# ucsdmanorlab/bootstrapper

Measured on AMD Instinct MI355X. Metric: Mvoxels/s predict+segment, 1024^3 vol in 128^3 blocks, higher is better.
Workload: dtype bf16x3

## Files before the change

### bootstrapper_amd/csrc/unet_api.hip

```cpp
#include <algorithm>
#include <cmath>
#include <cstdlib>
#include <cstring>
#include <map>
#include <memory>
#include <mutex>
#include <vector>
#include <chrono>
#include <thread>

#include "unet_internal.h"
#include "unet_ops.h"

#include "dev_guard.h"

namespace bsmi {

static thread_local std::string g_err;
void set_error(const char* fmt, ...) {
  char buf[1024];
  va_list ap;
  va_start(ap, fmt);
  vsnprintf(buf, sizeof buf, fmt, ap);
  va_end(ap);
// ... 170 lines not shown
        } else {
          const uint16_t hi = host_f32_to_bf16(v);
          const uint16_t lo = host_f32_to_bf16(v - host_bf16_to_f32(hi));
          uint16_t* w16 = (uint16_t*)packed.data();
          if (fused) {
            w16[idx] = hi;
            w16[idx + nelem] = lo;
          } else {
            const size_t blk = (size_t)pc.Npad * BKE;
            w16[idx] = hi;
            w16[idx + blk] = hi;
            w16[idx + 2 * blk] = lo;
          }
        }
      }
    }
  });
  BSMI_HIP(hipMalloc(&pc.w, packed.size()));
  BSMI_HIP(hipMemcpy(pc.w, packed.data(), packed.size(), hipMemcpyHostToDevice));
  BSMI_HIP(hipMalloc((void**)&pc.bias, bias.size() * sizeof(float)));
  BSMI_HIP(hipMemcpy(pc.bias, bias.data(), bias.size() * sizeof(float), hipMemcpyHostToDevice));
  pc.ready = true;
  return BSMI_OK;
}

static int wino_mode() {
  static const int m = [] { const char* e = getenv("BSMI_WINO"); return e ? atoi(e) : 1; }();
  return m;
}
static int wino4_mode();
static bool wino_eligible(const PassSite& p, int ci) {
  if (wino_mode() == 0 || p.k[ci][0] != 3 || p.k[ci][1] != 3 || p.k[ci][2] != 3) return false;
  if (ci == 0 && p.nslots > kWinoMaxSrc) return false;
  if (!x3_fused_for(choose_tile(p.cout))) return false;
  if (wino_mode() >= 2) return true;
  int cin = p.cout;
  if (ci == 0) {
    cin = 0;
    for (int s = 0; s < p.nslots; ++s) cin += p.cin[s];
  }
  if (cin >= 256 && p.cout >= 256) return true;
  return wino4_mode() == 1 && (int64_t)cin * p.cout >= 16384 && cin >= 32 && p.cout >= 32;
}

static int wino4_mode() {
  static const int m = [] { const char* e = getenv("BSMI_WINO4"); return e ? atoi(e) : 1; }();
  return m;
}
static int wino_tile_edge(const PassSite& p, int ci) {
  (void)p; (void)ci;
  return wino4_mode() == 0 ? 2 : 4;
}

static int pack_wino(bsmi_unet* h, PassSite& p, int ci) {
  PackedWino& pw = p.wino[ci];
  if (pw.w) { (void)hipFree(pw.w); pw.w = nullptr; }
  if (pw.res_w) { (void)hipFree(pw.res_w); pw.res_w = nullptr; }
  for (int part = 0; part < 2; ++part)
    if (pw.res_part_w[part]) { (void)hipFree(pw.res_part_w[part]); pw.res_part_w[part] = nullptr; }
  pw.ready = false;
  if (!wino_eligible(p, ci)) return BSMI_OK;
  const HostWeight& wm = h->weights[p.prefix + ".conv_pass." + std::to_string(2 * ci) + ".weight"];
  const HostWeight& wr = h->weights[p.prefix + ".residual.0.weight"];
  const int cin_m = (int)wm.shape[1];
  pw.cin_of_v.clear();
  if (ci == 0) {
    int base = 0;
    for (int s = 0; s < p.nslots; ++s) {
      for (int c = 0; c < round_up(p.cin[s], kChanPad); ++c) pw.cin_of_v.push_back(c < p.cin[s] ? base + c : -1);
      base += p.cin[s];
    }
  } else {
    for (int c = 0; c < round_up(p.cout, kChanPad); ++c) pw.cin_of_v.push_back(c < p.cout ? c : -1);
  }
  pw.Cv = (int)pw.cin_of_v.size();
  pw.m = wino_tile_edge(p, ci);
  pw.tile = choose_tile(p.cout);
  pw.Npad = round_up(p.cout, tile_bn(pw.tile));
  wino_units(pw.Cv, pw.units);
  {
    size_t image_elems = 0, batch_elems = 0;
    static const bool on_host = [] { const char* e = getenv("BSMI_WINO_PACK_HOST"); return e && e[0] == '1'; }();
    if (on_host) {
      std::vector<uint16_t> packed;
      wino_pack_weights(wm.data.data(), p.cout, cin_m, pw.cin_of_v, pw.Npad, pw.units, packed, image_elems, batch_elems, pw.m);
      BSMI_HIP(hipMalloc(&pw.w, packed.size() * 2));
      BSMI_HIP(hipMemcpy(pw.w, packed.data(), packed.size() * 2, hipMemcpyHostToDevice));
    } else {
      const int rc = wino_pack_weights_dev(wm.data.data(), p.cout, cin_m, pw.cin_of_v, pw.Npad, pw.units, pw.m, &pw.w, image_elems, batch_elems);
      if (rc) return rc;
    }
    pw.lo_image_bytes = image_elems * 2;
    pw.batch_bytes = batch_elems * 2;
  }
  pw.res_entries.clear();
  if (ci == p.nconv - 1) {
    std::vector<PackEntry> all;
    build_entries(p, ci, BSMI_PREC_BF16X3, all);
    for (size_t u = 0; u + 1 < all.size(); u += kUnitsPerStep) {
      bool res = false;
      for (int j = 0; j < kUnitsPerStep; ++j) res |= !all[u + j].dummy && all[u + j].wsrc == 1;
      if (res)
        for (int j = 0; j < kUnitsPerStep; ++j) pw.res_entries.push_back(all[u + j]);
    }
    if ((pw.res_entries.size() / kUnitsPerStep) % 2)
      for (int j = 0; j < kUnitsPerStep; ++j) pw.res_entries.push_back(PackEntry{0, 0, 0, 0, 0, 0, 0, 0, 0, true, 0});
    const int64_t cin_r = wr.shape[1];
    auto pack_res = [&](const std::vector<PackEntry>& ents, void** w_out, size_t* lo_out) -> int {
      const size_t nsteps = ents.size() / kUnitsPerStep;
      const size_t nelem = (nsteps * (size_t)pw.Npad + kWeightRowSlack) * 32;
      std::vector<uint16_t> packed(2 * nelem, 0);
      for (size_t u = 0; u < ents.size(); ++u) {
        const PackEntry& e = ents[u];
        if (e.dummy) continue;
// ... 403 lines not shown
            }
      }
    }
    const int n_full = (int)chunks.size();
    for (const Src& sr : center) {
      const TDesc& t = slots[sr.slot];
      const int org[3] = {so[sr.slot][0] + crop[0] / 2, so[sr.slot][1] + crop[1] / 2, so[sr.slot][2] + crop[2] / 2};
      for (int c0 = 0; c0 < t.Cpad; c0 += 32) {
        chunks.push_back(chunk_of(t, org, c0));
        const size_t w0 = wimg.size();
        wimg.resize(w0 + (size_t)NB * 64 * 4, 0u);
        for (int b = 0; b < NB; ++b)
          for (int l = 0; l < 64; ++l) {
            const int m = b * 16 + (l & 15), q = l >> 4;
            if (m >= p.cout) continue;
            for (int j = 0; j < 8; ++j) {
              const int c = c0 + q * 8 + j;
              if (c >= sr.creal) break;
              put(w0 + ((size_t)b * 64 + l) * 4, j, wr.data[(size_t)m * cin_r + (sr.cin_base + c)]);
            }
          }
      }
    }
    std::vector<float> bias((size_t)16 * NB, 0.f);
    for (int m = 0; m < p.cout; ++m) bias[m] = bm.data[m] + (last ? br.data[m] : 0.f);
    BoxChunk* dchunks = nullptr;
    uint32_t* dw = nullptr;
    float* dbias = nullptr;
    BSMI_HIP(hipMalloc((void**)&dchunks, chunks.size() * sizeof(BoxChunk)));
    plan->allocs.push_back(dchunks);
    BSMI_HIP(hipMalloc((void**)&dw, wimg.size() * 4));
    plan->allocs.push_back(dw);
    BSMI_HIP(hipMalloc((void**)&dbias, bias.size() * 4));
    plan->allocs.push_back(dbias);
    BSMI_HIP(hipMemcpy(dchunks, chunks.data(), chunks.size() * sizeof(BoxChunk), hipMemcpyHostToDevice));
    BSMI_HIP(hipMemcpy(dw, wimg.data(), wimg.size() * 4, hipMemcpyHostToDevice));
    BSMI_HIP(hipMemcpy(dbias, bias.data(), bias.size() * 4, hipMemcpyHostToDevice));
    st.box.chunks = dchunks;
    st.box.n_full = n_full;
    st.box.n_center = (int)chunks.size() - n_full;
    st.box.w = dw;
    st.box.bias = dbias;
    st.box.out = (uint16_t*)o.ptr;
    st.box.Do = o.D; st.box.Ho = o.H; st.box.Wo = o.W; st.box.Co = o.Cpad;
    st.use_box = true;
    (void)nsl;
    return BSMI_OK;
  }

  int plan_wino(PassSite& p, int ci, const PackedConv& pc, const TDesc* slots, const int (*so)[3], int nsl, const TDesc& o, PlanStep& st) {
    st.use_wino = false;
    const PackedWino& pw = p.wino[ci];
    const bool wants_fused = fuse_up && (ci == 0 || ci == p.nconv - 1);
    const int wm = pw.m, nbatch = wino_batches(wm);
    if (prec != BSMI_PREC_BF16X3 || !pw.ready || (wm == 2 && ((o.H & 1) || (o.W & 1))) || st.use_box || st.use_rh) {
      if (wants_fused) BSMI_FAIL(BSMI_ERR_STATE, "%s conv %d: the upsampling was fused into this stage, which cannot take the Winograd form", p.prefix.c_str(), ci);
      return BSMI_OK;
    }
    const int nsrc = ci == 0 ? p.nslots : 1;
    const int Dv = o.D + 2, Ty = (o.H + wm - 1) / wm, Tx = (o.W + wm - 1) / wm, Cv = pw.Cv;
    const size_t vbatch = (size_t)Dv * Ty * Tx * Cv * 4;
    if (vbatch >= ((size_t)1 << 31)) {
      if (wants_fused) BSMI_FAIL(BSMI_ERR_STATE, "%s conv %d: fused upsampling, but the transformed input is too large", p.prefix.c_str(), ci);
      return BSMI_OK;
    }
    const size_t Mrows = (size_t)o.D * Ty * Tx;
    void *V = nullptr, *Mbuf = nullptr, *addend = nullptr;
    BSMI_HIP(hipMalloc(&V, nbatch * vbatch + 4096));
    plan->allocs.push_back(V);
    BSMI_HIP(hipMalloc(&Mbuf, nbatch * Mrows * o.Cpad * sizeof(float)));
    plan->allocs.push_back(Mbuf);
    plan->bytes += nbatch * (vbatch + Mrows * o.Cpad * sizeof(float));
    WinoInArgs& wi = st.wino_in;
    memset(&wi, 0, sizeof wi);
    int cv0 = 0;
    for (int q = 0; q < nsrc; ++q) {
      const TDesc& t = slots[q];
      wi.src[q] = t.ptr;
      wi.H[q] = t.H; wi.W[q] = t.W; wi.Cpad[q] = t.Cpad;
      wi.oz[q] = so[q][0]; wi.oy[q] = so[q][1]; wi.ox[q] = so[q][2];
      wi.cv0[q] = cv0;
      cv0 += t.Cpad;
      if (fuse_up && ci == 0 && q == 1) {
        if (fuse_up->low.Cpad != t.Cpad) BSMI_FAIL(BSMI_ERR_STATE, "%s: fused upsampling with a different channel padding", p.prefix.c_str());
        wi.src[q] = fuse_up->low.ptr;
        wi.H[q] = fuse_up->low.H; wi.W[q] = fuse_up->low.W;
        wi.oz[q] += fuse_up->o[0]; wi.oy[q] += fuse_up->o[1]; wi.ox[q] += fuse_up->o[2];
        wi.upf[q] = fuse_up->f[1];
      }
    }
    if (cv0 != Cv) BSMI_FAIL(BSMI_ERR_STATE, "%s conv %d: winograd channel layout %d != %d", p.prefix.c_str(), ci, cv0, Cv);
    wi.nsrc = nsrc;
    wi.V = V;
    wi.Dv = Dv; wi.Ty = Ty; wi.Tx = Tx; wi.Cv = Cv;
    wi.m = wm;
    ConvArgs& g = st.wino_gemm;
    memset(&g, 0, sizeof g);
    for (int sl = 0; sl < kMaxConvTensors; ++sl) {
      g.t[sl].base = (uint64_t)(uintptr_t)V;
      g.t[sl].sz = (int32_t)((int64_t)Ty * Tx * Cv * 4);
      g.t[sl].sy = (int32_t)((int64_t)Tx * Cv * 4);
      g.t[sl].sx = (int32_t)((int64_t)Cv * 4);
    }
    {
      std::vector<KStep> ks(pw.units.size() / kUnitsPerStep);
      for (size_t s = 0; s < ks.size(); ++s) {
// ... 257 lines not shown
        }
        st.out = o;
        rc = plan_rh(p, ci, pc, slots, so, nsl, o, st);
        if (rc) return rc;
        rc = plan_box(p, ci, slots, so, nsl, o, st);
        if (rc) return rc;
        rc = plan_wino(p, ci, pc, slots, so, nsl, o, st);
        if (rc) return rc;
        if (!st.use_wino && !st.use_box) {
          rc = plan_h16(p, ci, pc, slots, so, o, st);
          if (rc) return rc;
        }
        if (getenv("BSMI_PLAN_DEBUG"))
          fprintf(stderr, "[bsmi plan] %s conv %d: out (%d,%d,%d)x%d tile BN=%d K-steps %d %s\n", p.prefix.c_str(), ci, o.D, o.H, o.W,
                  p.cout, tile_bn(st.tile), st.use_wino ? st.wino_gemm.nsteps : a.nsteps,
                  st.use_wino ? (st.wino_in.m == 4 ? "winograd F(4x4,3x3)" : "winograd F(2x2,3x3)") : st.use_h16 ? "halo-resident" : st.use_box ? "box-halo" : st.use_rh ? "raster-halo" : "gather");
        plan->steps.push_back(st);
      }
      cur = o;
      sp[0] = o.D; sp[1] = o.H; sp[2] = o.W;
    }
    out = cur;
    (void)crop;
    return BSMI_OK;
  }

  int rec(int level, const TDesc& f_in, TDesc& f_out) {
    const int i = h->nl - level - 1;
    TDesc f_left;
    const int org0[1][3] = {{0, 0, 0}};
    const int sp[3] = {f_in.D, f_in.H, f_in.W};
    int rc = pass(h->l_conv[i], &f_in, org0, sp, f_left);
    if (rc) return rc;
    if (level == 0) {
      f_out = f_left;
      return BSMI_OK;
    }
    const int* f = h->cfg.downsample_factors[i];
    const int dims[3] = {f_left.D, f_left.H, f_left.W};
    for (int d = 2; d >= 0; --d)
      if (dims[d] % f[d] != 0)
        BSMI_FAIL(BSMI_ERR_INVALID,
                  "Can not downsample shape (%d, %d, %d) with factor (%d, %d, %d), mismatch in spatial dimension %d",
                  dims[0], dims[1], dims[2], f[0], f[1], f[2], d);
    TDesc g_in;
    g_in.C = f_left.C; g_in.D = f_left.D / f[0]; g_in.H = f_left.H / f[1]; g_in.W = f_left.W / f[2];
    rc = alloc(g_in);
    if (rc) return rc;
    if (!dry) {
      PlanStep st;
      st.type = PlanStep::POOL;
      st.in = f_left; st.out = g_in;
      for (int d = 0; d < 3; ++d) st.f[d] = f[d];
      plan->steps.push_back(st);
    }
    TDesc g_out;
    rc = rec(level - 1, g_in, g_out);
    if (rc) return rc;

    PassSite& rp = h->r_conv[i];
    const int up[3] = {g_out.D * f[0], g_out.H * f[1], g_out.W * f[2]};
    int conv_crop[3] = {0, 0, 0};
    for (int c = 0; c < rp.nconv; ++c)
      for (int d = 0; d < 3; ++d) conv_crop[d] += rp.k[c][d] - 1;
    int target[3];
    for (int d = 0; d < 3; ++d) {
      const int cf = h->crop_factor[i][d];
      const int n = (int)std::floor((double)(up[d] - conv_crop[d]) / cf);
      target[d] = n * cf + conv_crop[d];
      if (target[d] != up[d] && target[d] <= conv_crop[d])
        BSMI_FAIL(BSMI_ERR_INVALID,
                  "Feature map with shape (%d, %d, %d) is too small to ensure translation equivariance",
                  up[0], up[1], up[2]);
    }
    TDesc g_c;
    g_c.C = g_out.C; g_c.D = target[0]; g_c.H = target[1]; g_c.W = target[2];
    rc = alloc(g_c);
    if (rc) return rc;
    int so[2][3];
    for (int d = 0; d < 3; ++d) {
      so[0][d] = (dims[d] - target[d]) / 2;
      so[1][d] = 0;
      if (dims[d] < target[d])
        BSMI_FAIL(BSMI_ERR_INVALID, "skip connection (%d,%d,%d) smaller than upsampled map (%d,%d,%d)",
                  dims[0], dims[1], dims[2], target[0], target[1], target[2]);
    }
    UpFuse uf;
    bool fuse = false;
    if (!dry && prec == BSMI_PREC_BF16X3 && f[0] == 1 && f[1] == 2 && f[2] == 2 && rp.nslots == 2 && rp.wino[0].ready &&
        rp.wino[rp.nconv - 1].ready && !rp.wino[rp.nconv - 1].res_part[1].empty() && g_out.ptr) {
      static const bool on = [] { const char* e = getenv("BSMI_FUSE_UP"); return !(e && e[0] == '0'); }();
      fuse = on;
      int sp[3] = {target[0], target[1], target[2]};
      for (int c = 0; c < rp.nconv && fuse; ++c) {
        for (int d = 0; d < 3; ++d) sp[d] -= rp.k[c][d] - 1;
        const int wm = rp.wino[c].m;
        if ((c == 0 || c == rp.nconv - 1) && ((wm == 2 && ((sp[1] & 1) || (sp[2] & 1))) || sp[0] <= 0 || sp[1] <= 0 || sp[2] <= 0)) fuse = false;
        if ((c == 0 || c == rp.nconv - 1) && (size_t)(sp[0] + 2) * ((sp[1] + wm - 1) / wm) * ((sp[2] + wm - 1) / wm) * rp.wino[c].Cv * 4 >= ((size_t)1 << 31)) fuse = false;
      }
    }
    size_t up_index = 0;
    if (!dry) {
      PlanStep st;
      st.type = PlanStep::UP;
      st.in = g_out; st.out = g_c;
      for (int d = 0; d < 3; ++d) { st.f[d] = f[d]; st.o[d] = (up[d] - target[d]) / 2; }
// ... 19 lines not shown
    x.C = h->cfg.in_channels; x.D = (int)in_shape[0]; x.H = (int)in_shape[1]; x.W = (int)in_shape[2];
    int rc = alloc(x);
    if (rc) return rc;
    if (!dry) {
      PlanStep st;
      st.type = PlanStep::INPUT;
      st.out = x;
      plan->steps.push_back(st);
    }
    TDesc z;
    rc = rec(h->nl - 1, x, z);
    if (rc) return rc;
    plan->out_shape[0] = z.D; plan->out_shape[1] = z.H; plan->out_shape[2] = z.W;
    for (size_t hd = 0; hd < h->heads.size(); ++hd) {
      plan->flops += 2.0 * 2.0 * (double)z.D * z.H * z.W * h->heads[hd].cin * h->heads[hd].cout;
      if (!dry) {
        PlanStep st;
        st.type = PlanStep::HEAD;
        st.in = z;
        st.head = (int)hd;
        st.flops = 2.0 * 2.0 * (double)z.D * z.H * z.W * h->heads[hd].cin * h->heads[hd].cout;
        plan->steps.push_back(st);
      }
    }
    return BSMI_OK;
  }
};

static void free_plan(Plan* p) {
  for (void* a : p->allocs) (void)hipFree(a);
  p->allocs.clear();
  for (auto* sets : {&p->inflight, &p->spare})
    for (auto& set : *sets)
      for (hipEvent_t e : set) (void)hipEventDestroy(e);
  p->inflight.clear();
  p->spare.clear();
  p->events.clear();
}

static int harvest(bsmi_unet* h, Plan* plan) {
  if (!plan || plan->inflight.empty()) return BSMI_OK;
  const size_t n = plan->steps.size();
  for (auto& set : plan->inflight) {
    plan->last_ms.assign(n, 0.f);
    BSMI_HIP(hipEventSynchronize(set[2 * n - 1]));
    for (size_t i = 0; i < n; ++i) {
      float t = 0.f;
      BSMI_HIP(hipEventElapsedTime(&t, set[2 * i], set[2 * i + 1]));
      plan->last_ms[i] = t;
      const int ty = (plan->fused_first && i < 2) ? (int)PlanStep::CONV : (int)plan->steps[i].type;
      h->prof_ms[ty] += t;
      h->prof_flops[ty] += plan->steps[i].flops;
      if (ty == 1) h->prof_exec += plan->steps[i].exec_flops > 0 ? plan->steps[i].exec_flops : plan->steps[i].flops * (plan->prec == BSMI_PREC_BF16X3 ? 3.0 : 1.0);
      h->prof_launches[ty] += (plan->fused_first && i < 2) ? 0 : 1;
    }
    plan->spare.push_back(std::move(set));
  }
  plan->inflight.clear();
  plan->pending = false;
  return BSMI_OK;
}

namespace {
std::mutex g_chain_mu;
struct ChainState { hipEvent_t done = nullptr; hipStream_t last = nullptr; bool any = false; };
ChainState g_chain[16];
}
struct ForwardChain {
  std::unique_lock<std::mutex> lock{g_chain_mu};
};
static bool forward_chain_on() {
  static const bool on = [] { const char* e = getenv("BSMI_FORWARD_CHAIN"); return e && e[0] == '1'; }();
  return on;
}
static int forward_chain_enter(int device, hipStream_t s) {
  if (device < 0 || device >= 16 || !forward_chain_on()) return BSMI_OK;
  ChainState& c = g_chain[device];
  if (c.any && c.last != s) BSMI_HIP(hipStreamWaitEvent(s, c.done, 0));
  return BSMI_OK;
}
static int forward_chain_leave(int device, hipStream_t s) {
  if (device < 0 || device >= 16 || !forward_chain_on()) return BSMI_OK;
  ChainState& c = g_chain[device];
  if (!c.done) BSMI_HIP(hipEventCreateWithFlags(&c.done, hipEventDisableTiming));
  BSMI_HIP(hipEventRecord(c.done, s));
  c.last = s;
  c.any = true;
  return BSMI_OK;
}

static bool first_pass_eligible(const bsmi_unet* h) {
  if (h->cfg.in_channels != 1 || h->l_conv.empty()) return false;
  const PassSite& p = h->l_conv[0];
  if (p.nconv != 2 || p.cout > 16) return false;
  for (int c = 0; c < 2; ++c)
    for (int d = 0; d < 3; ++d)
      if (p.k[c][d] != 3) return false;
  const char* e = getenv("BSMI_FUSED_FIRST");
  return !(e && e[0] == '0');
}

int get_plan(bsmi_unet* h, int precision, const int64_t in_shape[3], Plan** out) {
  const std::vector<int64_t> key = {precision, in_shape[0], in_shape[1], in_shape[2]};
  auto it = h->plans.find(key);
  if (it == h->plans.end()) {
    std::unique_ptr<Plan> plan(new Plan);
    plan->prec = precision;
    Planner pl{h, precision, plan.get(), false};
    const int rc = pl.run(in_shape);
    if (rc) {
      free_plan(plan.get());
      return rc;
    }
    const std::vector<PlanStep>& ps = plan->steps;
    const bool fp_ready = precision == BSMI_PREC_BF16 ? h->first_pass.ready : precision == BSMI_PREC_BF16X3 && h->first_pass_x3.ready;
    plan->fused_first = fp_ready && first_pass_eligible(h) && ps.size() > 3 &&
                        ps[0].type == PlanStep::INPUT && ps[1].type == PlanStep::CONV && ps[2].type == PlanStep::CONV &&
                        ps[1].site == &h->l_conv[0] && ps[2].site == &h->l_conv[0] && ps[2].out.Cpad == 16;
    BSMI_HIP(hipDeviceSynchronize());
    it = h->plans.emplace(key, std::move(plan)).first;
  }
  *out = it->second.get();
  return BSMI_OK;
}

static int check_shape_arg(const int64_t s[3]) {
  for (int d = 0; d < 3; ++d)
    if (s[d] <= 0 || s[d] > 4096) BSMI_FAIL(BSMI_ERR_INVALID, "bad input shape (%lld,%lld,%lld)", (long long)s[0], (long long)s[1], (long long)s[2]);
  return BSMI_OK;
}

}

extern "C" {

const char* bsmi_last_error(void) { return g_err.c_str(); }
int bsmi_version(void) { return 1; }

int bsmi_unet_create(const bsmi_unet_config* cfg, int device, bsmi_unet** out) {
  if (!cfg || !out) BSMI_FAIL(BSMI_ERR_INVALID, "null argument");
  if (cfg->num_levels < 1 || cfg->num_levels > BSMI_MAX_LEVELS) BSMI_FAIL(BSMI_ERR_INVALID, "num_levels %d out of range", cfg->num_levels);
  if (cfg->num_heads < 1 || cfg->num_heads > BSMI_MAX_HEADS) BSMI_FAIL(BSMI_ERR_INVALID, "num_heads %d out of range", cfg->num_heads);
  if (cfg->in_channels < 1 || cfg->num_fmaps < 1 || cfg->fmap_inc_factor < 1 || cfg->num_fmaps_out < 0) BSMI_FAIL(BSMI_ERR_INVALID, "bad channel configuration");
  std::unique_ptr<bsmi_unet> h(new bsmi_unet);
  h->cfg = *cfg;
  h->device = device;
  h->nl = cfg->num_levels;
  auto fm = [&](int level) {
    int64_t c = cfg->num_fmaps;
    for (int i = 0; i < level; ++i) c *= cfg->fmap_inc_factor;
    return (int)c;
  };
  auto fill_k = [&](PassSite& p, int n, const int32_t (*k)[3]) -> int {
    if (n < 1 || n > BSMI_MAX_CONVS) BSMI_FAIL(BSMI_ERR_INVALID, "%s: %d convolutions per pass unsupported", p.prefix.c_str(), n);
    p.nconv = n;
    for (int i = 0; i < n; ++i)
      for (int d = 0; d < 3; ++d) {
        if (k[i][d] < 1 || k[i][d] > 7) BSMI_FAIL(BSMI_ERR_INVALID, "%s: kernel size %d unsupported", p.prefix.c_str(), k[i][d]);
        p.k[i][d] = k[i][d];
      }
    return BSMI_OK;
  };
  for (int l = 0; l < h->nl; ++l) {
    PassSite p;
    p.prefix = "unet.l_conv." + std::to_string(l);
    p.nslots = 1;
    p.cin[0] = l == 0 ? cfg->in_channels : fm(l - 1);
    p.cout = fm(l);
    int rc = fill_k(p, cfg->n_convs_down[l], cfg->kernel_size_down[l]);
    if (rc) return rc;
    h->l_conv.push_back(p);
// ... 264 lines not shown
    const char* e = getenv("BSMI_STREAMK");
    if ((e && e[0] == '0') || h->sk_request == 0) {
      h->sk_grid = -1;
    } else {
      hipDeviceProp_t prop;
      BSMI_HIP(hipGetDeviceProperties(&prop, h->device));
      h->sk_grid = h->sk_request >= 0 ? h->sk_request : prop.multiProcessorCount / 8 * 8;
      if (const char* g = getenv("BSMI_SK_GRID")) h->sk_grid = std::max(8, atoi(g) / 8 * 8);
      BSMI_HIP(hipMalloc((void**)&h->sk_ws, stream_k_ws_bytes(h->sk_grid)));
      BSMI_HIP(hipMemsetAsync((char*)h->sk_ws + stream_k_ws_bytes(h->sk_grid) - 64, 0, 64, s));
    }
  }
  if (h->train && precision == BSMI_PREC_F32 && !h->train_forward && (rc = train_refresh_f32_images(h, s))) return rc;
  size_t step_idx = 0;
  for (const PlanStep& st : plan.steps) {
    if (prof) BSMI_HIP(hipEventRecord(plan.events[2 * step_idx], s));
    if (plan.fused_first && step_idx < 3) {
      if (step_idx == 2) {
        FirstPassArgs fa;
        fa.raw = raw_dev; fa.raw_dtype = raw_dtype;
        fa.D = plan.steps[0].out.D; fa.H = plan.steps[0].out.H; fa.W = plan.steps[0].out.W;
        fa.out = (uint16_t*)st.out.ptr;
        const FirstPassWeights& fw = precision == BSMI_PREC_BF16X3 ? h->first_pass_x3 : h->first_pass;
        fa.w1a = fw.w1a; fa.w2a = fw.w2a; fa.vec = fw.vec;
        fa.split = fw.split;
        rc = launch_first_pass(fa, h->sk_grid > 0 ? h->sk_grid : 256, s);
        if (rc) return rc;
      }
      if (prof) BSMI_HIP(hipEventRecord(plan.events[2 * step_idx + 1], s));
      ++step_idx;
      continue;
    }
    switch (st.type) {
      case PlanStep::INPUT:
        rc = launch_input_prep(precision, raw_dev, raw_dtype, st.out.ptr, st.out.C, st.out.Cpad,
                               (size_t)st.out.D * st.out.H * st.out.W, s);
        break;
      case PlanStep::CONV:
        if (st.use_wino && !(st.tx3 && h->train_forward)) {
          if ((rc = launch_wino_in(st.wino_in, s))) break;
          if ((rc = launch_conv_igemm(st.wino_gemm, precision, st.tile, s, h->sk_ws, h->sk_grid))) break;
          if (st.wino_has_res && (rc = launch_conv_igemm(st.wino_res, precision, st.tile, s, h->sk_ws, h->sk_grid))) break;
          if (st.wino_has_res_low && (rc = launch_conv_igemm(st.wino_res_low, precision, st.tile, s, h->sk_ws, h->sk_grid))) break;
          rc = launch_wino_out(st.wino_out, s);
          break;
        }
        rc = (st.tx3 && h->train_forward) ? train_forward_conv_x3(h, st, s)
             : st.use_h16 ? launch_conv_h16(st.h16, st.h16_rows, s)
             : st.use_box ? launch_conv_box(st.box, s)
             : st.use_rh ? launch_conv_rh(st.rh, precision, st.tile, s, h->sk_ws, h->sk_grid)
                         : launch_conv_igemm(st.conv, precision, st.tile, s, h->sk_ws, h->sk_grid);
        break;
      case PlanStep::POOL:
        rc = launch_maxpool(precision, st.in.ptr, st.out.ptr, st.in.D, st.in.H, st.in.W, st.in.Cpad,
                            st.f[0], st.f[1], st.f[2], s);
        break;
      case PlanStep::UP:
        if (st.skip) break;
        rc = launch_upsample_crop(precision, st.in.ptr, st.out.ptr, st.in.D, st.in.H, st.in.W, st.in.Cpad,
                                  st.out.D, st.out.H, st.out.W, st.f[0], st.f[1], st.f[2], st.o[0], st.o[1], st.o[2], s);
        break;
      case PlanStep::HEAD: {
        const HeadSite& hd = h->heads[st.head];
        float* of = out_f32_dev ? out_f32_dev[st.head] : nullptr;
        uint8_t* ou = out_u8_dev ? out_u8_dev[st.head] : nullptr;
        if (of || ou)
          rc = launch_head(precision, st.in.ptr, st.in.Cpad, hd.cin, hd.cout, hd.hw, hd.hb, of, ou,
                           (size_t)st.in.D * st.in.H * st.in.W, s);
        break;
      }
    }
    if (rc) return rc;
    if (prof) BSMI_HIP(hipEventRecord(plan.events[2 * step_idx + 1], s));
    ++step_idx;
  }
  if (prof) plan.inflight.push_back(std::move(plan.events));
  return forward_chain_leave(h->device, s);
}

int bsmi_unet_debug_activation(bsmi_unet* h, int step, int what, int64_t shape_out[4], float* host_out, uint64_t capacity) {
  if (!h || !shape_out) BSMI_FAIL(BSMI_ERR_INVALID, "null argument");
  Plan* plan = h->last_plan;
  if (!plan) BSMI_FAIL(BSMI_ERR_STATE, "no forward has run");
  if (step < 0 || step >= (int)plan->steps.size()) BSMI_FAIL(BSMI_ERR_INVALID, "step %d out of range (%zu steps)", step, plan->steps.size());
  const PlanStep& st = plan->steps[step];
  if (st.type == PlanStep::HEAD) BSMI_FAIL(BSMI_ERR_INVALID, "head steps write into the caller's buffers");
  if (plan->fused_first && step < 2)
    BSMI_FAIL(BSMI_ERR_STATE, "step %d is not materialised: the first ConvPass ran as one launch (first_pass), which writes step 2 only", step);
  if (st.type == PlanStep::UP && st.skip)
    BSMI_FAIL(BSMI_ERR_STATE, "step %d is not materialised: the upsampling is fused into the Winograd stages that read it", step);
  const TDesc& t = st.out;
  shape_out[0] = t.D; shape_out[1] = t.H; shape_out[2] = t.W; shape_out[3] = t.C;
  if (!host_out) return BSMI_OK;
  const size_t nvox = (size_t)t.D * t.H * t.W;
  if (capacity < nvox * t.C) BSMI_FAIL(BSMI_ERR_INVALID, "buffer of %llu floats too small", (unsigned long long)capacity);
  BSMI_HIP(hipSetDevice(h->device));
  BSMI_HIP(hipDeviceSynchronize());
  const int es = esize(plan->prec);
  const bool split = t.lo_off != 0;
  const size_t bytes = nvox * t.Cpad * es * (split ? 2 : 1);
  std::vector<uint8_t> raw(bytes);
  BSMI_HIP(hipMemcpy(raw.data(), t.ptr, raw.size(), hipMemcpyDeviceToHost));
  for (size_t v = 0; v < nvox; ++v)
    for (int c = 0; c < t.C; ++c) {
      float x;
      if (plan->prec == BSMI_PREC_F32) {
// ... 130 lines not shown
```

### bootstrapper_amd/csrc/unet_internal.h

```cpp
#pragma once
#include <map>
#include <memory>
#include <string>
#include <vector>

#include "conv_igemm.h"
#include "conv_rh.h"
#include "conv_h16.h"
#include "conv_box.h"
#include "first_pass.h"
#include "wino.h"

namespace bsmi {

struct HostWeight {
  std::vector<int64_t> shape;
  std::vector<float> data;
  bool loaded = false;
};

struct PackEntry {
  int slot;
  int dz, dy, dx;
  int c0;
  int wsrc;
  int tap;
  int cin_base;
  int creal;
  bool dummy;
  int phase;
};

struct PackPhase {
  int slot, c0, kind, first_unit, nunits;
};

struct PackedConv {
  bool ready = false;
  std::vector<PackEntry> entries;
  std::vector<PackPhase> phases;
  void* w = nullptr;
  int ks = 1;
  size_t lo_image_bytes = 0;
  float* bias = nullptr;
  int Npad = 0;
  TileCfg tile = TILE_256x32;
};

struct PackedWino {
  bool ready = false;
  int m = 2;
  std::vector<WinoUnit> units;
  std::vector<int> cin_of_v;
  int Cv = 0;
  void* w = nullptr;
  size_t lo_image_bytes = 0, batch_bytes = 0;
  int Npad = 0;
  TileCfg tile = TILE_256x32;
  std::vector<PackEntry> res_entries;
  void* res_w = nullptr;
  size_t res_lo_image_bytes = 0;
  std::vector<PackEntry> res_part[2];
  void* res_part_w[2] = {nullptr, nullptr};
  size_t res_part_lo[2] = {0, 0};
};

struct H16PhaseHost {
  int slot, c0, dz, kind;
  int first_step, nsteps;
};
struct PackedH16 {
  bool ready = false;
  std::vector<PackEntry> entries;
  std::vector<H16PhaseHost> phases;
  void* w = nullptr;
  size_t lo_image_bytes = 0;
  int Npad = 0;
};

struct PassSite {
  std::string prefix;
  int nslots = 1;
  int cin[2] = {0, 0};
  int cout = 0;
  int nconv = 0;
  int k[BSMI_MAX_CONVS][3];
  PackedConv packed[BSMI_NUM_PREC][BSMI_MAX_CONVS];
  PackedWino wino[BSMI_MAX_CONVS];
  PackedH16 h16[BSMI_MAX_CONVS];
};

struct HeadSite {
  std::string prefix;
  int cin = 0, cout = 0;
  float* hw = nullptr;
  float* hb = nullptr;
};

struct TDesc {
  void* ptr = nullptr;
  int C = 0, Cpad = 0, D = 0, H = 0, W = 0;
  size_t lo_off = 0;
};

struct PlanStep {
  enum Type { INPUT, CONV, POOL, UP, HEAD } type;
  ConvArgs conv;
  RhArgs rh;
  bool use_rh = false;
  H16Args h16;
  bool use_h16 = false;
  int h16_rows = 0;
  BoxArgs box;
  bool use_box = false;
  bool use_wino = false;
  WinoInArgs wino_in;
  ConvArgs wino_gemm, wino_res, wino_res_low;
  bool wino_has_res = false, wino_has_res_low = false;
  WinoOutArgs wino_out;
  TileCfg tile;
  TDesc in, out;
  int f[3], o[3];
  bool skip = false;
  int head = 0;
  double flops = 0;
  double exec_flops = 0;
  struct PassSite* site = nullptr;
  int ci = 0;
  TDesc slots[kMaxConvTensors];
  int so[kMaxConvTensors][3] = {{0, 0, 0}, {0, 0, 0}, {0, 0, 0}};
  int nsl = 0;
  struct TrainFwdX3* tx3 = nullptr;
};

struct Plan {
  std::vector<float> last_ms;
  bool pending = false;
  std::vector<void*> allocs;
  std::vector<PlanStep> steps;
  int64_t out_shape[3] = {0, 0, 0};
  double flops = 0;
  size_t bytes = 0;
  std::vector<hipEvent_t> events;
  std::vector<std::vector<hipEvent_t>> inflight, spare;
  bool profiled = false;
  bool fused_first = false;
  int prec = 0;
};

struct TrainState;

int esize(int prec);
int ksplit(int prec);
int bke(int prec);
int sube(int prec);
void build_entries(const PassSite& p, int ci, int prec, std::vector<PackEntry>& out, std::vector<PackPhase>* phases_out = nullptr);

}

using namespace bsmi;

struct bsmi_unet {
  bsmi_unet_config cfg;
  int device = 0;
  int nl = 0;
  std::vector<PassSite> l_conv, r_conv;
  std::vector<HeadSite> heads;
  int crop_factor[BSMI_MAX_LEVELS][3];
  std::map<std::string, HostWeight> weights;
  bool finalized[BSMI_NUM_PREC] = {false, false, false};
  int profile_period = 0;
  uint64_t profile_count = 0;
  Plan* last_plan = nullptr;
  double prof_ms[5] = {0, 0, 0, 0, 0}, prof_flops[5] = {0, 0, 0, 0, 0};
  double prof_exec = 0;
  int64_t prof_launches[5] = {0, 0, 0, 0, 0};
// ... 19 lines not shown
```

### bootstrapper_amd/csrc/wino.h

```cpp
#pragma once
#include <vector>

#include "conv_igemm.h"

namespace bsmi {

constexpr int kWinoBatch = 16;
constexpr int kWinoMaxBatch = 36;
inline int wino_batches(int m) { return (m + 2) * (m + 2); }
constexpr int kWinoMaxSrc = 2;

struct WinoInArgs {
  const void* src[kWinoMaxSrc];
  int H[kWinoMaxSrc], W[kWinoMaxSrc], Cpad[kWinoMaxSrc];
  int oz[kWinoMaxSrc], oy[kWinoMaxSrc], ox[kWinoMaxSrc];
  int cv0[kWinoMaxSrc];
  int upf[kWinoMaxSrc];
  int nsrc;
  void* V;
  int Dv, Ty, Tx, Cv;
  int m;
};

struct WinoOutArgs {
  const float* M;
  const float* addend;
  const float* low;
  int lD, lH, lW, lf, loz, loy, lox;
  const float* bias;
  void* out;
  int Do, Ty, Tx, Co;
  int relu;
  int m, Ho, Wo;
};

int launch_wino_in(const WinoInArgs& a, hipStream_t s);
int launch_wino_out(const WinoOutArgs& a, hipStream_t s);

struct WinoUnit {
  int kz, vc0;
  bool dummy;
};
void wino_units(int Cv, std::vector<WinoUnit>& out);

void wino_pack_weights(const float* w, int cout, int cin, const std::vector<int>& cin_of_v, int Npad, const std::vector<WinoUnit>& units,
                       std::vector<uint16_t>& packed, size_t& image_elems, size_t& batch_elems, int m = 2);

int wino_pack_weights_dev(const float* w, int cout, int cin, const std::vector<int>& cin_of_v, int Npad, const std::vector<WinoUnit>& units, int m,
                          void** image_dev, size_t& image_elems, size_t& batch_elems);

}
```

### bootstrapper_amd/csrc/wino.hip

```cpp
#include "wino.h"

#include <cstdlib>
#include <cstring>

#include "dev_guard.h"

namespace bsmi {

typedef uint32_t u32x4_t __attribute__((ext_vector_type(4)));
typedef float f32x4_t __attribute__((ext_vector_type(4)));

namespace {

__device__ __forceinline__ uint16_t to_bf16(float f) {
  __bf16 h = (__bf16)f;
  return __builtin_bit_cast(uint16_t, h);
}
__device__ __forceinline__ void unpack8(u32x4_t v, float* f) {
  const uint32_t w[4] = {v.x, v.y, v.z, v.w};
#pragma unroll
  for (int i = 0; i < 4; ++i) {
    f[2 * i] = __uint_as_float(w[i] << 16);
    f[2 * i + 1] = __uint_as_float(w[i] & 0xffff0000u);
  }
// ... 454 lines not shown
  const size_t e_out = (((size_t)z * a.Ty + ty) * a.Tx) * a.Cv + a.cv0[src] + 8 * cv;
  float ct[5][6][4];
  auto load_ct = [&](int c, int xlow) __attribute__((always_inline)) {
    const int x = xlow < 0 ? 0 : (xlow > W - 1 ? W - 1 : xlow);
    float L[5][4];
#pragma unroll
    for (int k = 0; k < 5; ++k) load_split4(sp, e_low + ((size_t)wy[k] * W + x) * C, hf, L[k]);
#pragma unroll
    for (int xi = 0; xi < 6; ++xi)
#pragma unroll
      for (int ch = 0; ch < 4; ++ch) {
        float acc = 0.f;
#pragma unroll
        for (int k = 0; k < 5; ++k)
          if (tu4(PY, xi, k) != 0.f) acc += tu4(PY, xi, k) * L[k][ch];
        ct[c][xi][ch] = acc;
      }
  };
  load_ct(0, bx + 2 * tx0);
  load_ct(1, bx + 2 * tx0 + 1);
  load_ct(2, bx + 2 * tx0 + 2);
  uint16_t* vt = (uint16_t*)a.V + 2 * (e_out + (size_t)tx0 * a.Cv) + 8 * hf;
  for (int tx = tx0; tx < tx1; ++tx) {
    load_ct(3, bx + 2 * tx + 3);
    load_ct(4, bx + 2 * tx + 4);
    uint16_t* vp = vt;
#pragma unroll
    for (int xi = 0; xi < 6; ++xi) {
#pragma unroll
      for (int nu = 0; nu < 6; ++nu) {
        float v[4];
#pragma unroll
        for (int ch = 0; ch < 4; ++ch) {
          float acc = 0.f;
#pragma unroll
          for (int c = 0; c < 5; ++c)
            if (tu4(PX, nu, c) != 0.f) acc += tu4(PX, nu, c) * ct[c][xi][ch];
          v[ch] = acc;
        }
        store_split4_pair(vp, hf, v);
        vp += 2 * plane;
      }
    }
    vt += 2 * a.Cv;
#pragma unroll
    for (int c = 0; c < 3; ++c)
#pragma unroll
      for (int xi = 0; xi < 6; ++xi)
#pragma unroll
        for (int ch = 0; ch < 4; ++ch) ct[c][xi][ch] = ct[c + 2][xi][ch];
  }
}

template <bool LOW>
__global__ __launch_bounds__(256) void wino4_out_kernel(const WinoOutArgs a, size_t total) {
  const size_t i = (size_t)blockIdx.x * blockDim.x + threadIdx.x;
  if (i >= total) return;
  const int ncg = a.Co >> 2;
  const int cg = (int)(i % ncg), cv = cg >> 1, hf = cg & 1;
  size_t t = i / ncg;
  const int tx = (int)(t % a.Tx);
  t /= a.Tx;
  const int ty = (int)(t % a.Ty);
  const int z = (int)(t / a.Ty);
  const size_t Mrows = (size_t)a.Do * a.Ty * a.Tx;
  const size_t m = ((size_t)z * a.Ty + ty) * a.Tx + tx;
  float tp[6][4][4];
#pragma unroll
  for (int nu = 0; nu < 6; ++nu) {
    float mm[6][4];
#pragma unroll
    for (int xi = 0; xi < 6; ++xi) {
      const f32x4_t v = __builtin_nontemporal_load((const f32x4_t*)(a.M + ((size_t)(6 * xi + nu) * Mrows + m) * a.Co + 4 * cg));
#pragma unroll
      for (int k = 0; k < 4; ++k) mm[xi][k] = v[k];
    }
    at4_apply(mm, tp[nu]);
  }
  float bv[4];
#pragma unroll
  for (int k = 0; k < 4; ++k) bv[k] = a.bias[4 * cg + k];
  uint16_t* out = (uint16_t*)a.out;
#pragma unroll
  for (int p = 0; p < 4; ++p) {
    float in[6][4], y[4][4];
#pragma unroll
    for (int nu = 0; nu < 6; ++nu)
#pragma unroll
      for (int k = 0; k < 4; ++k) in[nu][k] = tp[nu][p][k];
    at4_apply(in, y);
    const int oy = 4 * ty + p;
    if (oy >= a.Ho) continue;
#pragma unroll
    for (int q = 0; q < 4; ++q) {
      const int ox = 4 * tx + q;
      if (ox >= a.Wo) continue;
      const size_t e8 = (((size_t)z * a.Ho + oy) * a.Wo + ox) * a.Co + 8 * cv;
      const size_t e = e8 + 4 * hf;
      float v[4];
#pragma unroll
      for (int k = 0; k < 4; ++k) v[k] = y[q][k] + bv[k];
      if (a.addend) {
        const f32x4_t r0 = __builtin_nontemporal_load((const f32x4_t*)(a.addend + e));
#pragma unroll
        for (int k = 0; k < 4; ++k) v[k] += r0[k];
      }
      if constexpr (LOW) {
        int y0, y1, x0, x1;
        float wy0, wy1, wx0, wx1;
        lin_src(oy + a.loy, a.lf, a.lH, y0, y1, wy0, wy1);
        lin_src(ox + a.lox, a.lf, a.lW, x0, x1, wx0, wx1);
        const float* base = a.low + ((size_t)(z + a.loz) * a.lH * a.lW) * a.Co + 4 * cg;
        const f32x4_t r00 = *(const f32x4_t*)(base + ((size_t)y0 * a.lW + x0) * a.Co), r01 = *(const f32x4_t*)(base + ((size_t)y0 * a.lW + x1) * a.Co);
        const f32x4_t r10 = *(const f32x4_t*)(base + ((size_t)y1 * a.lW + x0) * a.Co), r11 = *(const f32x4_t*)(base + ((size_t)y1 * a.lW + x1) * a.Co);
#pragma unroll
        for (int k = 0; k < 4; ++k) {
          const float pa = wx0 * r00[k] + wx1 * r01[k];
          const float pb = wx0 * r10[k] + wx1 * r11[k];
          v[k] += wy0 * pa + wy1 * pb;
        }
      }
      if (a.relu) {
#pragma unroll
        for (int k = 0; k < 4; ++k) v[k] = v[k] > 0.f ? v[k] : 0.f;
      }
      store_split4(out, e8, hf, v);
    }
  }
}

}

static int wino_in_seg_mode() {
  static const int m = [] { const char* e = getenv("BSMI_WINO_IN_SEG"); return e ? atoi(e) : -1; }();
  return m;
}
static void wino_in_segments(int Tx, int& S, int& nseg) {
  const int mode = wino_in_seg_mode();
  S = mode < 0 ? 1 : mode == 0 ? Tx : mode < Tx ? mode : Tx;
  nseg = (Tx + S - 1) / S;
}

int launch_wino_in(const WinoInArgs& a, hipStream_t s) {
  const int m = a.m == 4 ? 4 : 2;
  if (a.m != 0 && a.m != 2 && a.m != 4) BSMI_FAIL(BSMI_ERR_INVALID, "winograd input transform: tile edge %d (2 or 4)", a.m);
  if (a.nsrc < 1 || a.nsrc > kWinoMaxSrc || a.Dv <= 0 || a.Ty <= 0 || a.Tx <= 0 || a.Cv % 8) BSMI_FAIL(BSMI_ERR_INVALID, "winograd input transform: bad geometry");
  for (int q = 0; q < a.nsrc; ++q) {
    if (a.Cpad[q] % 8 || a.cv0[q] % 8 || a.cv0[q] + a.Cpad[q] > a.Cv) BSMI_FAIL(BSMI_ERR_INVALID, "winograd input transform: bad channel layout of source %d", q);
    const int upf = a.upf[q] > 0 ? a.upf[q] : 1;
    if (m == 2 && (a.oy[q] + 2 * a.Ty + 2 > a.H[q] * upf || a.ox[q] + 2 * a.Tx + 2 > a.W[q] * upf)) BSMI_FAIL(BSMI_ERR_INVALID, "winograd input transform: tiles leave source %d", q);
    if (m == 4 && (a.oy[q] < 0 || a.ox[q] < 0 || a.oy[q] + 4 * a.Ty + 2 > a.H[q] * upf + 3 || a.ox[q] + 4 * a.Tx + 2 > a.W[q] * upf + 3))
      BSMI_FAIL(BSMI_ERR_INVALID, "winograd input transform: F(4x4) tiles leave source %d by more than a tile's overhang", q);
    int S = a.Tx, nseg = 1;
    if (m == 4) wino_in_segments(a.Tx, S, nseg);
    const size_t total = (size_t)a.Dv * a.Ty * (a.Cpad[q] / (m == 4 ? 4 : 8)) * nseg;
    const dim3 grid((unsigned)((total + 255) / 256));
    if (a.upf[q] > 0) {
      if (a.upf[q] != 2 || a.oy[q] < 0 || a.ox[q] < 0) BSMI_FAIL(BSMI_ERR_INVALID, "winograd input transform: only a factor-2 upsampling can be fused");
      const int par = 2 * (a.oy[q] & 1) + (a.ox[q] & 1);
      if (m == 4) {
        if (par == 0) hipLaunchKernelGGL((wino4_in_up_kernel<0, 0>), grid, dim3(256), 0, s, a, q, total, S, nseg);
        else if (par == 1) hipLaunchKernelGGL((wino4_in_up_kernel<0, 1>), grid, dim3(256), 0, s, a, q, total, S, nseg);
        else if (par == 2) hipLaunchKernelGGL((wino4_in_up_kernel<1, 0>), grid, dim3(256), 0, s, a, q, total, S, nseg);
        else hipLaunchKernelGGL((wino4_in_up_kernel<1, 1>), grid, dim3(256), 0, s, a, q, total, S, nseg);
      } else if (par == 0) hipLaunchKernelGGL((wino_in_up_kernel<0, 0>), grid, dim3(256), 0, s, a, q, total);
      else if (par == 1) hipLaunchKernelGGL((wino_in_up_kernel<0, 1>), grid, dim3(256), 0, s, a, q, total);
      else if (par == 2) hipLaunchKernelGGL((wino_in_up_kernel<1, 0>), grid, dim3(256), 0, s, a, q, total);
      else hipLaunchKernelGGL((wino_in_up_kernel<1, 1>), grid, dim3(256), 0, s, a, q, total);
    } else if (m == 4) {
      hipLaunchKernelGGL(wino4_in_kernel, grid, dim3(256), 0, s, a, q, total, S, nseg);
    } else {
      hipLaunchKernelGGL(wino_in_kernel, grid, dim3(256), 0, s, a, q, total);
    }
  }
  BSMI_HIP(hipGetLastError());
  return BSMI_OK;
}

int launch_wino_out(const WinoOutArgs& a, hipStream_t s) {
  const int m = a.m == 4 ? 4 : 2;
  if (a.m != 0 && a.m != 2 && a.m != 4) BSMI_FAIL(BSMI_ERR_INVALID, "winograd output transform: tile edge %d (2 or 4)", a.m);
  if (a.Do <= 0 || a.Ty <= 0 || a.Tx <= 0 || a.Co % 8) BSMI_FAIL(BSMI_ERR_INVALID, "winograd output transform: bad geometry");
  const int Ho = m == 4 ? a.Ho : 2 * a.Ty, Wo = m == 4 ? a.Wo : 2 * a.Tx;
  if (m == 4 && (Ho < 1 || Wo < 1 || Ho > 4 * a.Ty || Wo > 4 * a.Tx || Ho + 3 < 4 * a.Ty || Wo + 3 < 4 * a.Tx)) BSMI_FAIL(BSMI_ERR_INVALID, "winograd output transform: output extent and F(4x4) tile counts disagree");
  if (a.low && (a.lf < 1 || a.loz < 0 || a.loz + a.Do > a.lD || a.loy < 0 || a.loy + Ho > a.lH * a.lf || a.lox < 0 || a.lox + Wo > a.lW * a.lf))
    BSMI_FAIL(BSMI_ERR_INVALID, "winograd output transform: the low-resolution residual does not cover the output");
  const size_t total = (size_t)a.Do * a.Ty * a.Tx * (a.Co / (m == 4 ? 4 : 8));
  const dim3 grid((unsigned)((total + 255) / 256));
  if (m == 4) {
    if (a.low) hipLaunchKernelGGL(wino4_out_kernel<true>, grid, dim3(256), 0, s, a, total);
    else hipLaunchKernelGGL(wino4_out_kernel<false>, grid, dim3(256), 0, s, a, total);
  } else if (a.low) hipLaunchKernelGGL(wino_out_kernel<true>, grid, dim3(256), 0, s, a, total);
  else hipLaunchKernelGGL(wino_out_kernel<false>, grid, dim3(256), 0, s, a, total);
  BSMI_HIP(hipGetLastError());
  return BSMI_OK;
}

void wino_units(int Cv, std::vector<WinoUnit>& out) {
  out.clear();
  for (int c32 = 0; c32 < Cv; c32 += 32)
    for (int kz = 0; kz < 3; ++kz)
      for (int j = 0; j < kUnitsPerStep; ++j) {
        const int c = c32 + 16 * j;
        if (c < Cv) out.push_back(WinoUnit{kz, c, false});
        else out.push_back(WinoUnit{0, 0, true});
      }
  if ((out.size() / kUnitsPerStep) % 2)
    for (int j = 0; j < kUnitsPerStep; ++j) out.push_back(WinoUnit{0, 0, true});
}

static inline uint16_t host_bf16(float f) {
  uint32_t u;
  memcpy(&u, &f, 4);
  if ((u & 0x7fffffffu) > 0x7f800000u) return (uint16_t)((u >> 16) | 0x40);
  u += 0x7fffu + ((u >> 16) & 1u);
  return (uint16_t)(u >> 16);
}
static inline float host_bf16_f32(uint16_t b) {
  const uint32_t u = (uint32_t)b << 16;
  float f;
  memcpy(&f, &u, 4);
  return f;
}

void wino_pack_weights(const float* w, int cout, int cin, const std::vector<int>& cin_of_v, int Npad, const std::vector<WinoUnit>& units,
                       std::vector<uint16_t>& packed, size_t& image_elems, size_t& batch_elems, int m) {
  const size_t nsteps = units.size() / kUnitsPerStep;
  const int T = m + 2, nbatch = T * T;
  batch_elems = nsteps * (size_t)Npad * 32;
  image_elems = nbatch * batch_elems + (size_t)kWeightRowSlack * 32;
  packed.assign(2 * image_elems, 0);
  static const double G2[4][3] = {{1, 0, 0}, {.5, .5, .5}, {.5, -.5, .5}, {0, 0, 1}};
  const double a = 0.70710678118654752440, b = 1.41421356237309504880;
  const double G4[6][3] = {{1, 0, 0}, {2. / 3, 2. / 3 * a, 1. / 3}, {2. / 3, -2. / 3 * a, 1. / 3}, {1. / 12, b / 12, 1. / 6}, {1. / 12, -b / 12, 1. / 6}, {0, 0, 1}};
  double G[6][3];
  for (int i = 0; i < T; ++i)
    for (int k = 0; k < 3; ++k) G[i][k] = m == 4 ? G4[i][k] : G2[i][k];
  host_parallel_for((size_t)cout, [&](size_t n_) {
    const int n = (int)n_;
    for (size_t u = 0; u < units.size(); ++u) {
      const WinoUnit& un = units[u];
      if (un.dummy) continue;
      const size_t s = u / kUnitsPerStep, j = u % kUnitsPerStep;
// ... 116 lines not shown
```

Before: 105.8.

## Fuse 1x2x2 max-pool into Winograd F(4x4) output transform and enable narrow last conv Winograd

After: 108.9, median of 6. 3.0% higher.

```diff
diff --git a/bootstrapper_amd/csrc/unet_api.hip b/bootstrapper_amd/csrc/unet_api.hip
--- a/bootstrapper_amd/csrc/unet_api.hip
+++ b/bootstrapper_amd/csrc/unet_api.hip
@@ -246,6 +246,19 @@
   return wino4_mode() == 0 ? 2 : 4;
 }
 
+static bool fuse_up_narrow() {
+  static const bool on = [] { const char* e = getenv("BSMI_FUSE_UP_NARROW"); return !(e && e[0] == '0'); }();
+  return on;
+}
+static bool wino_narrow_last(const bsmi_unet* h, const PassSite& p, int ci) {
+  if (!fuse_up_narrow() || wino_mode() == 0 || p.nslots != 2 || p.nconv < 2 || ci != p.nconv - 1) return false;
+  if (&p < h->r_conv.data() || &p >= h->r_conv.data() + h->r_conv.size()) return false;
+  const int* f = h->cfg.downsample_factors[&p - h->r_conv.data()];
+  if (f[0] != 1 || f[1] != 2 || f[2] != 2) return false;
+  if (p.k[ci][0] != 3 || p.k[ci][1] != 3 || p.k[ci][2] != 3 || p.cout < 32 || !x3_fused_for(choose_tile(p.cout))) return false;
+  return wino_eligible(p, 0) && !wino_eligible(p, ci);
+}
+
 static int pack_wino(bsmi_unet* h, PassSite& p, int ci) {
   PackedWino& pw = p.wino[ci];
   if (pw.w) { (void)hipFree(pw.w); pw.w = nullptr; }
@@ -253,7 +266,8 @@
   for (int part = 0; part < 2; ++part)
     if (pw.res_part_w[part]) { (void)hipFree(pw.res_part_w[part]); pw.res_part_w[part] = nullptr; }
   pw.ready = false;
-  if (!wino_eligible(p, ci)) return BSMI_OK;
+  pw.fused_only = wino_narrow_last(h, p, ci);
+  if (!wino_eligible(p, ci) && !pw.fused_only) return BSMI_OK;
   const HostWeight& wm = h->weights[p.prefix + ".conv_pass." + std::to_string(2 * ci) + ".weight"];
   const HostWeight& wr = h->weights[p.prefix + ".residual.0.weight"];
   const int cin_m = (int)wm.shape[1];
@@ -763,6 +777,7 @@
     st.use_wino = false;
     const PackedWino& pw = p.wino[ci];
     const bool wants_fused = fuse_up && (ci == 0 || ci == p.nconv - 1);
+    if (pw.fused_only && !fuse_up) return BSMI_OK;
     const int wm = pw.m, nbatch = wino_batches(wm);
     if (prec != BSMI_PREC_BF16X3 || !pw.ready || (wm == 2 && ((o.H & 1) || (o.W & 1))) || st.use_box || st.use_rh) {
       if (wants_fused) BSMI_FAIL(BSMI_ERR_STATE, "%s conv %d: the upsampling was fused into this stage, which cannot take the Winograd form", p.prefix.c_str(), ci);
@@ -1126,6 +1141,13 @@
       st.type = PlanStep::POOL;
       st.in = f_left; st.out = g_in;
       for (int d = 0; d < 3; ++d) st.f[d] = f[d];
+      static const bool pool_fuse = [] { const char* e = getenv("BSMI_POOL_FUSE"); return !(e && e[0] == '0'); }();
+      PlanStep& prod = plan->steps.back();
+      if (pool_fuse && prec == BSMI_PREC_BF16X3 && f[0] == 1 && f[1] == 2 && f[2] == 2 && prod.type == PlanStep::CONV && prod.use_wino &&
+          prod.wino_out.m == 4 && !prod.wino_out.low && prod.wino_out.out == f_left.ptr && !(f_left.H & 1) && !(f_left.W & 1)) {
+        prod.wino_out.pool = g_in.ptr;
+        st.pool_fused = true;
+      }
       plan->steps.push_back(st);
     }
     TDesc g_out;
@@ -1251,7 +1273,7 @@
       h->prof_ms[ty] += t;
       h->prof_flops[ty] += plan->steps[i].flops;
       if (ty == 1) h->prof_exec += plan->steps[i].exec_flops > 0 ? plan->steps[i].exec_flops : plan->steps[i].flops * (plan->prec == BSMI_PREC_BF16X3 ? 3.0 : 1.0);
-      h->prof_launches[ty] += (plan->fused_first && i < 2) ? 0 : 1;
+      h->prof_launches[ty] += ((plan->fused_first && i < 2) || plan->steps[i].pool_fused) ? 0 : 1;
     }
     plan->spare.push_back(std::move(set));
   }
@@ -1316,6 +1338,10 @@
     plan->fused_first = fp_ready && first_pass_eligible(h) && ps.size() > 3 &&
                         ps[0].type == PlanStep::INPUT && ps[1].type == PlanStep::CONV && ps[2].type == PlanStep::CONV &&
                         ps[1].site == &h->l_conv[0] && ps[2].site == &h->l_conv[0] && ps[2].out.Cpad == 16;
+    if (plan->fused_first && plan->steps[3].type == PlanStep::POOL && plan->steps[3].pool_fused) {
+      plan->steps[3].pool_fused = false;
+      plan->steps[2].wino_out.pool = nullptr;
+    }
     BSMI_HIP(hipDeviceSynchronize());
     it = h->plans.emplace(key, std::move(plan)).first;
   }
@@ -1686,6 +1712,7 @@
                          : launch_conv_igemm(st.conv, precision, st.tile, s, h->sk_ws, h->sk_grid);
         break;
       case PlanStep::POOL:
+        if (st.pool_fused) break;
         rc = launch_maxpool(precision, st.in.ptr, st.out.ptr, st.in.D, st.in.H, st.in.W, st.in.Cpad,
                             st.f[0], st.f[1], st.f[2], s);
         break;
diff --git a/bootstrapper_amd/csrc/unet_internal.h b/bootstrapper_amd/csrc/unet_internal.h
--- a/bootstrapper_amd/csrc/unet_internal.h
+++ b/bootstrapper_amd/csrc/unet_internal.h
@@ -50,6 +50,7 @@
 struct PackedWino {
   bool ready = false;
   int m = 2;
+  bool fused_only = false;
   std::vector<WinoUnit> units;
   std::vector<int> cin_of_v;
   int Cv = 0;
@@ -122,6 +123,7 @@
   TDesc in, out;
   int f[3], o[3];
   bool skip = false;
+  bool pool_fused = false;
   int head = 0;
   double flops = 0;
   double exec_flops = 0;
diff --git a/bootstrapper_amd/csrc/wino.h b/bootstrapper_amd/csrc/wino.h
--- a/bootstrapper_amd/csrc/wino.h
+++ b/bootstrapper_amd/csrc/wino.h
@@ -32,6 +32,7 @@
   int Do, Ty, Tx, Co;
   int relu;
   int m, Ho, Wo;
+  void* pool;
 };
 
 int launch_wino_in(const WinoInArgs& a, hipStream_t s);
diff --git a/bootstrapper_amd/csrc/wino.hip b/bootstrapper_amd/csrc/wino.hip
--- a/bootstrapper_amd/csrc/wino.hip
+++ b/bootstrapper_amd/csrc/wino.hip
@@ -530,7 +530,7 @@
   }
 }
 
-template <bool LOW>
+template <bool LOW, bool POOL = false>
 __global__ __launch_bounds__(256) void wino4_out_kernel(const WinoOutArgs a, size_t total) {
   const size_t i = (size_t)blockIdx.x * blockDim.x + threadIdx.x;
   if (i >= total) return;
@@ -559,6 +559,7 @@
 #pragma unroll
   for (int k = 0; k < 4; ++k) bv[k] = a.bias[4 * cg + k];
   uint16_t* out = (uint16_t*)a.out;
+  [[maybe_unused]] float even[4][4];
 #pragma unroll
   for (int p = 0; p < 4; ++p) {
     float in[6][4], y[4][4];
@@ -569,6 +570,7 @@
     at4_apply(in, y);
     const int oy = 4 * ty + p;
     if (oy >= a.Ho) continue;
+    [[maybe_unused]] float left[4];
 #pragma unroll
     for (int q = 0; q < 4; ++q) {
       const int ox = 4 * tx + q;
@@ -603,6 +605,27 @@
         for (int k = 0; k < 4; ++k) v[k] = v[k] > 0.f ? v[k] : 0.f;
       }
       store_split4(out, e8, hf, v);
+      if constexpr (POOL) {
+        float sv[4];
+#pragma unroll
+        for (int k = 0; k < 4; ++k) {
+          const float h = __uint_as_float((uint32_t)to_bf16(v[k]) << 16);
+          sv[k] = h + __uint_as_float((uint32_t)to_bf16(v[k] - h) << 16);
+        }
+        if ((p & 1) == 0) {
+#pragma unroll
+          for (int k = 0; k < 4; ++k) even[q][k] = sv[k];
+        } else if ((q & 1) == 0) {
+#pragma unroll
+          for (int k = 0; k < 4; ++k) left[k] = sv[k];
+        } else {
+          float mx[4];
+#pragma unroll
+          for (int k = 0; k < 4; ++k) mx[k] = fmaxf(fmaxf(fmaxf(fmaxf(-INFINITY, even[q > 0 ? q - 1 : 0][k]), even[q][k]), left[k]), sv[k]);
+          const size_t pe = (((size_t)z * (a.Ho >> 1) + (oy >> 1)) * (a.Wo >> 1) + (ox >> 1)) * a.Co + 8 * cv;
+          store_split4((uint16_t*)a.pool, pe, hf, mx);
+        }
+      }
     }
   }
 }
@@ -661,12 +684,14 @@
   if (a.Do <= 0 || a.Ty <= 0 || a.Tx <= 0 || a.Co % 8) BSMI_FAIL(BSMI_ERR_INVALID, "winograd output transform: bad geometry");
   const int Ho = m == 4 ? a.Ho : 2 * a.Ty, Wo = m == 4 ? a.Wo : 2 * a.Tx;
   if (m == 4 && (Ho < 1 || Wo < 1 || Ho > 4 * a.Ty || Wo > 4 * a.Tx || Ho + 3 < 4 * a.Ty || Wo + 3 < 4 * a.Tx)) BSMI_FAIL(BSMI_ERR_INVALID, "winograd output transform: output extent and F(4x4) tile counts disagree");
+  if (a.pool && (m != 4 || a.low || (Ho & 1) || (Wo & 1))) BSMI_FAIL(BSMI_ERR_INVALID, "winograd output transform: a pooled output needs F(4x4), even extents and no low-resolution residual");
   if (a.low && (a.lf < 1 || a.loz < 0 || a.loz + a.Do > a.lD || a.loy < 0 || a.loy + Ho > a.lH * a.lf || a.lox < 0 || a.lox + Wo > a.lW * a.lf))
     BSMI_FAIL(BSMI_ERR_INVALID, "winograd output transform: the low-resolution residual does not cover the output");
   const size_t total = (size_t)a.Do * a.Ty * a.Tx * (a.Co / (m == 4 ? 4 : 8));
   const dim3 grid((unsigned)((total + 255) / 256));
   if (m == 4) {
     if (a.low) hipLaunchKernelGGL(wino4_out_kernel<true>, grid, dim3(256), 0, s, a, total);
+    else if (a.pool) hipLaunchKernelGGL((wino4_out_kernel<false, true>), grid, dim3(256), 0, s, a, total);
     else hipLaunchKernelGGL(wino4_out_kernel<false>, grid, dim3(256), 0, s, a, total);
   } else if (a.low) hipLaunchKernelGGL(wino_out_kernel<true>, grid, dim3(256), 0, s, a, total);
   else hipLaunchKernelGGL(wino_out_kernel<false>, grid, dim3(256), 0, s, a, total);
```
